# rossumur/espflix

Measured on AMD Instinct MI355X. Metric: MPEG-1 352x192 frames/s, higher is better.
Workload: dtype u8/int32; 1 GPU; 1024 streams/GPU x GOP(12) I+11P, 352x192 MPEG-1 ES resident in HBM, ids rank*1024.. per rank (BASELINE configs[2]; at 8 GPUs = configs[4], stream k on rank floor(k*8/8192)); streams_per_gpu=1024, streams_total=1024, es_bytes_per_gpu=46457181, parallelism=stream-partition x1, coefficients_per_gpu=44531885, ring_depth=2

## Files before the change

espflix_amd/csrc/efx_api.hip:

```cpp
#include <hip/hip_runtime.h>

#include <algorithm>
#include <memory>
#include <mutex>
#include <thread>

#include <cstdio>
#include <cstdlib>
#include <cstring>
#include <string>
#include <vector>

#include "efx.h"
#include "conform_sel.h"
#include "efx_internal.h"
#include "enc_core.h"
#include "import_px.h"
#include "crop_px.h"
#include "parse_tm.h"
#include "sbc_enc_core.h"
#include "trick_sel.h"

namespace efx {
struct DemuxChunk;
__global__ void k_demux_scan(const uint8_t*, const uint64_t*, const uint32_t*, const uint32_t*, DemuxChunk*);
__global__ void k_demux_offsets(const uint32_t*, const uint32_t*, DemuxChunk*, uint8_t*, const uint64_t*, uint32_t*, uint32_t*);
__global__ void k_demux(const uint8_t*, const uint64_t*, const uint32_t*, const uint32_t*, const DemuxChunk*, uint8_t*, PesEntry*);
__global__ void k_demux_fused(const uint8_t*, const uint64_t*, const uint32_t*, const uint32_t*, DemuxChunk*, uint8_t*, PesEntry*, uint32_t*, uint32_t*,
                              uint32_t*);
__global__ void k_demux_audio_scan(const uint8_t*, const uint64_t*, const uint32_t*, const uint32_t*, DemuxChunk*);
__global__ void k_demux_audio_offsets(const uint32_t*, const uint32_t*, DemuxChunk*, uint32_t*);
__global__ void k_demux_audio(const uint8_t*, const uint64_t*, const uint32_t*, const uint32_t*, const DemuxChunk*, uint8_t*, const uint64_t*);
__global__ void k_ts_sequences(const uint8_t*, const uint64_t*, const uint32_t*, const uint32_t*, PesEntry*, IdxInfo*);
__global__ void k_idx_bins(const PesEntry*, const uint32_t*, const IdxInfo*, uint32_t, uint32_t*, size_t);
__global__ void k_index(const uint8_t*, const uint64_t*, int, PicInfo*, SliceTmp*, uint32_t*, uint32_t*, uint32_t*,
                        const uint32_t*, const PesEntry*, const uint32_t*, const uint32_t*, int64_t*, int64_t*, int, int, int);
__global__ void k_advance(StreamState*, const uint32_t*, int64_t*, const int64_t*, int, int, int, int32_t*);
__global__ void k_slice_scan(const PicInfo*, const uint32_t*, int, int, const uint32_t*, uint32_t*, DecodeCounters*);
__global__ void k_slice_emit(const PicInfo*, const SliceTmp*, const uint32_t*, const uint64_t*, const uint32_t*, int, int,
                             const uint32_t*, SliceDesc*, uint32_t*);
__global__ void k_parse(const uint8_t*, const SliceDesc*, DecodeCounters*, const TmTables*, MbRec*, TmU4*, uint32_t*, uint32_t*,
                        int, int);
__global__ void k_recon(const MbRec*, const uint32_t*, const uint32_t*, const uint32_t*, uint8_t*, int, int, int, const int32_t*, int, int);
__global__ void k_recon_all(const MbRec*, const uint32_t*, const uint32_t*, const uint32_t*, uint8_t*, int, int, int, const int32_t*, int, int,
                            int, uint32_t*, uint32_t*, int);

__global__ void k_frame_hash(const uint8_t*, int, uint64_t*);
__global__ void k_fill(uint32_t*, uint32_t, size_t);
__global__ void k_composite(const uint8_t*, const VideoTables*, const VideoLineTemplates*, FieldArgs, uint16_t*);
__global__ void k_pdm(const int16_t*, int, int, int32_t*, uint16_t*);
template <int FMT, int CHROMA>
__global__ void k_export(const uint8_t*, int, ExportArgs);
__global__ void k_import_taps(ImportTap*, ImportArgs);
__global__ void k_import(const uint8_t*, uint8_t*, const ImportTap*, ImportArgs);
__global__ void k_crop_zero(CropArgs);
__global__ void k_crop_sums_i420(CropArgs);
__global__ void k_crop_sums_rgb24(CropArgs);
__global__ void k_crop_sums_rgbp(CropArgs);
__global__ void k_crop_rects(CropArgs);
template <int SOURCE>
__global__ void k_trick(TrickArgs);
__global__ void k_conform(ConformArgs);
__global__ void k_import_pcm(ImportPcmArgs);
__global__ void k_import_pcm_state(ImportPcmArgs);
__global__ void k_enc_begin(EncArgs);
__global__ void k_enc_act(EncArgs);
__global__ void k_enc_rows(EncArgs);
__global__ void k_enc_pack(EncArgs);
__global__ void k_sbc(const uint8_t*, size_t, int, int, SbcState*, const SbcTables*, int16_t*, size_t, uint32_t*, uint32_t*, int);
__global__ void k_sbc_frames(const uint8_t*, size_t, int, int, SbcFrameInfo*, uint32_t*, uint32_t*, SbcQueues*);
__global__ void k_sbc_plan(const SbcFrameInfo*, int, int, const SbcState*, SbcFramePlan*, uint32_t*, SbcQueues*, uint32_t*, int, int, uint32_t*,
                           uint32_t*, SbcExtraItem*, uint8_t*);
__global__ void k_sbc_par_stereo(const uint8_t*, size_t, int, int, const SbcState*, SbcState*, const SbcTables*, const SbcFrameInfo*, int16_t*,
                                 size_t, uint32_t*, int, SbcQueues*, const uint32_t*, int, const SbcExtraItem*, int);
__global__ void k_sbc_par_mono(const uint8_t*, size_t, int, int, const SbcState*, SbcState*, const SbcTables*, const SbcFrameInfo*, int16_t*,
                               size_t, uint32_t*, int, SbcQueues*, const uint32_t*, int, const SbcExtraItem*, int);
__global__ void k_sbc_gen(const uint8_t*, size_t, int, int, const SbcState*, SbcState*, const SbcTables*, const SbcFrameInfo*,
                          const SbcFramePlan*, int16_t*, size_t, int, SbcQueues*, const uint32_t*, int, const uint8_t*, int);
__global__ void k_sbc_finish(const uint8_t*, size_t, int, int, SbcState*, const SbcState*, const SbcTables*, int16_t*, size_t, uint32_t*,
                             uint32_t*, int, uint32_t*);
__global__ void k_sbc_enc(SbcEncArgs);
__global__ void k_sbc_enc_state(SbcEncArgs);
__global__ void k_mux(MuxArgs);
}

using namespace efx;

#ifndef EFX_SBC_WG_PER_CU
#define EFX_SBC_WG_PER_CU 4
#endif

#ifndef EFX_PARSE_STREAMS
#define EFX_PARSE_STREAMS 2
#endif
#ifndef EFX_SLOTS
#define EFX_SLOTS 3
#endif
constexpr int kParseStreams = EFX_PARSE_STREAMS;
constexpr int kMaxGroups = 16;
static_assert(kMaxGroups <= kExportMaxGroups, "k_export takes every reconstruction group of a call");
#ifndef EFX_RECON_MERGE
#define EFX_RECON_MERGE 1
#endif
constexpr int kReconMerge = EFX_RECON_MERGE;
#ifndef EFX_GROUP_STREAMS
#define EFX_GROUP_STREAMS 1024
#endif
constexpr int kGroupStreams = EFX_GROUP_STREAMS;
constexpr int kTimingRing = 64;
constexpr int kSlots = EFX_SLOTS;
constexpr int kUploads = 3;
constexpr size_t kReconSyncWords(size_t streams) { return (64 + streams) * 32; }

struct efx_ctx {
    efx_config cfg{};
    hipStream_t stream = nullptr;
    bool own_stream = false;
    bool pooled_streams = false;
    unsigned stream_serial = 0;
    std::string err;

    size_t es_cap = 0;
    bool decoded = false, results_valid = false;

    ParseTables* d_tables = nullptr;
    TmTables* d_tm_tables = nullptr;
    uint8_t* d_frames = nullptr;
    StreamState* d_state = nullptr;

    struct Upload {
        uint8_t* d_es = nullptr;
        uint64_t* d_stream_off = nullptr;
        uint32_t* d_stream_perm = nullptr;
        uint32_t* d_ts_len = nullptr;
        uint32_t* d_pkt_base = nullptr;
        uint32_t* d_es_len = nullptr;
        uint32_t* d_pes_count = nullptr;
        PesEntry* d_pes = nullptr;
        uint8_t* h_es = nullptr;
        uint8_t* h_meta = nullptr;
        std::vector<uint64_t> stream_off;
        std::vector<uint32_t> es_len;
        int n_streams = 0;
        int sort_groups = 1;
        size_t es_used = 0, ts_bytes = 0;
        bool ts_input = false, valid = false;
        hipEvent_t uploaded = nullptr;
        hipEvent_t last_read[kParseStreams] = {};
        hipEvent_t ev_demux[2] = {nullptr, nullptr};
        bool demux_timed = false;
    } up[kUploads];
    int cur_up = -1;
    struct Arena {
        uint8_t* base;
        size_t bytes;
        bool owned;
    };
    std::vector<Arena> arenas;
    hipStream_t copy_stream = nullptr;
    uint8_t* d_ts = nullptr;
    DemuxChunk* d_demux_chunks = nullptr;
    size_t pes_cap = 0;
    IdxInfo* d_idx_info = nullptr;
    uint64_t* d_ts_off = nullptr;
    uint32_t* d_idx_len = nullptr;
    uint32_t* d_idx_base = nullptr;
    PesEntry* d_idx_seq = nullptr;
    bool ts_ready = false;

    struct Slot {
        uint32_t* d_pic_count = nullptr;
        uint32_t* d_status = nullptr;
        DecodeCounters* d_counters = nullptr;
// ... 955 lines not shown
    bind_device(ctx);
    if (!ctx)
        return EFX_ERR_ARG;
    const size_t n = (size_t)ctx->cfg.max_streams;
    EFX_HIP(hipMemsetAsync(ctx->d_frames, 0, n * ctx->cfg.ring_depth * kFrameBytes, ctx->stream));
    std::vector<StreamState> init(n);
    for (auto& st : init) {
        st.fb_index = 1;
        st.pts_seen = 0;
        st.pts_carry = -1;
    }
    EFX_HIP(hipMemcpyAsync(ctx->d_state, init.data(), n * sizeof(StreamState), hipMemcpyHostToDevice, ctx->stream));
    EFX_HIP(hipStreamSynchronize(ctx->stream));
    ctx->recon_groups_unsynced = 0;
    return EFX_OK;
}

int efx_play_reset(efx_ctx* ctx)
{
    bind_device(ctx);
    if (!ctx)
        return EFX_ERR_ARG;
    int r = sync_all(ctx);
    if (r)
        return r;
    const size_t n = (size_t)ctx->cfg.max_streams;
    std::vector<StreamState> st(n);
    EFX_HIP(hipMemcpy(st.data(), ctx->d_state, n * sizeof(StreamState), hipMemcpyDeviceToHost));
    for (auto& x : st)
        x.pts_seen = 0;
    EFX_HIP(hipMemcpy(ctx->d_state, st.data(), n * sizeof(StreamState), hipMemcpyHostToDevice));
    return EFX_OK;
}

int efx_stream_state(efx_ctx* ctx, int stream, uint32_t* frame_index, int* pts_seen, int64_t* newest_pts)
{
    bind_device(ctx);
    if (!ctx || stream < 0 || stream >= ctx->cfg.max_streams)
        return EFX_ERR_ARG;
    int r = sync_all(ctx);
    if (r)
        return r;
    StreamState st;
    EFX_HIP(hipMemcpy(&st, ctx->d_state + stream, sizeof(st), hipMemcpyDeviceToHost));
    if (frame_index)
        *frame_index = st.fb_index;
    if (pts_seen)
        *pts_seen = (int)st.pts_seen;
    if (newest_pts)
        *newest_pts = st.pts_carry;
    return EFX_OK;
}

int efx_erase_frames(efx_ctx* ctx)
{
    bind_device(ctx);
    if (!ctx)
        return EFX_ERR_ARG;
    size_t bytes = (size_t)ctx->cfg.max_streams * ctx->cfg.ring_depth * kFrameBytes;
    EFX_HIP(hipMemsetAsync(ctx->d_frames, 0x30, bytes, ctx->stream));
    return EFX_OK;
}

int efx_decode_from(efx_ctx* ctx, int first_picture) { return efx_decode_range(ctx, first_picture, ctx ? ctx->cfg.max_pictures : 0); }

int efx_decode_range(efx_ctx* ctx, int first_picture, int n_pictures)
{
    bind_device(ctx);
    if (!ctx || first_picture < 0 || n_pictures < 1 || n_pictures > ctx->cfg.max_pictures)
        return EFX_ERR_ARG;
    if (ctx->cur_up < 0)
        return fail(ctx, EFX_ERR_STATE, "efx_decode: no streams uploaded");
    efx_ctx::Upload& u = ctx->up[ctx->cur_up];
    const int n_all = u.n_streams, P = ctx->cfg.max_pictures, D = ctx->cfg.ring_depth;
    const bool idle_at_call = ctx->recon_groups_unsynced == 0;
    const int G = ctx->opt_groups > 0 ? std::min(std::min(ctx->opt_groups, kMaxGroups), std::max(1, n_all / 8))
                                      : (idle_at_call ? group_count(n_all) : 1);
    {
        bool nested = true;
        for (int g = 1; g < G && nested; g++) {
            bool found = false;
            for (int k = 0; k <= u.sort_groups && !found; k++)
                found = group_first(n_all, u.sort_groups, k) == group_first(n_all, G, g);
            nested = found;
        }
        if (!nested) {
            int r = sync_all(ctx);
            if (r)
                return r;
            std::vector<uint32_t> perm((size_t)n_all);
            for (int i = 0; i < n_all; i++)
                perm[i] = (uint32_t)i;
            auto len_of = [&](uint32_t i) { return u.stream_off[i + 1] - u.stream_off[i]; };
            for (int g = 0; g < G; g++)
                std::stable_sort(perm.begin() + group_first(n_all, G, g), perm.begin() + group_first(n_all, G, g + 1),
                                 [&](uint32_t a, uint32_t b) { return len_of(a) > len_of(b); });
            EFX_HIP(hipMemcpy(u.d_stream_perm, perm.data(), perm.size() * sizeof(uint32_t), hipMemcpyHostToDevice));
            u.sort_groups = G;
        }
    }
    hipStream_t sr = ctx->stream;
    int timing_slot = -1;
    if (ctx->timing && !ctx->timing_ring.empty()) {
        timing_slot = (int)(ctx->timed_calls++ % kTimingRing);
        ctx->timing_groups[timing_slot] = (uint8_t)G;
        ctx->timing_leaders[timing_slot] = 0;
        ctx->timing_launches[timing_slot] = (uint16_t)(((G + kReconMerge - 1) / kReconMerge) * (ctx->opt_recon_mode == 0 ? n_pictures : 1));
    }
    ctx->last_upload = ctx->cur_up;
    ctx->last_n_streams = u.n_streams;
    ctx->last_ts_input = u.ts_input;
    const int R = (G + kReconMerge - 1) / kReconMerge;
    ctx->n_groups = R;
    for (int r = 0; r < R; r++) {
        const int h0 = r * kReconMerge, h1 = std::min(G, h0 + kReconMerge);
        const int rs0 = group_first(n_all, G, h0), rn = group_first(n_all, G, h1) - rs0;
        const int slot = (int)(ctx->subcalls++ % kSlots);
        ctx->groups[r] = {slot, rs0, rn, h0, h1 - h0};
        efx_ctx::Slot& sl = ctx->slot[slot];
        sl.upload = ctx->cur_up;
        const bool wrap = ++sl.epoch > 255;
        if (wrap)
            sl.epoch = 1;
        efx_ctx::TimingEvents* te0 = nullptr;
        for (int g = h0; g < h1; g++) {
            const int s0 = group_first(n_all, G, g), n = group_first(n_all, G, g + 1) - s0;
            const int pi = (int)(ctx->parse_calls++ % kParseStreams);
            hipStream_t sp = ctx->parse_streams[pi];
            DecodeCounters* counters = sl.d_counters + g;
            uint32_t* slice_base = sl.d_slice_base + (size_t)s0 * P + g;
            SliceDesc* descs = sl.d_descs + (size_t)s0 * P * kMaxSlicesPerPicture;

            EFX_HIP(hipStreamWaitEvent(sp, u.uploaded, 0));
            EFX_HIP(hipStreamWaitEvent(sp, sl.recon_done, 0));
            if (wrap && g == h0) {
                EFX_HIP(hipMemsetAsync(sl.d_mbrecs, 0, (size_t)ctx->cfg.max_streams * P * kMbCount * sizeof(MbRec), sp));
                EFX_HIP(hipEventRecord(sl.wrap_cleared, sp));
            } else if (wrap)
                EFX_HIP(hipStreamWaitEvent(sp, sl.wrap_cleared, 0));
            efx_ctx::TimingEvents* te = timing_slot >= 0 ? &ctx->timing_ring[(size_t)timing_slot * kMaxGroups + g] : nullptr;
            if (te && !te->ev[0])
                for (auto& ev : te->ev)
                    EFX_HIP(hipEventCreate(&ev));
            if (g == h0)
                te0 = te;
            if (te)
                EFX_HIP(hipEventRecord(te->ev[0], sp));
            hipLaunchKernelGGL(k_index, dim3(n), dim3(64 * kIndexWaves), 0, sp, u.d_es, u.d_stream_off, P, sl.d_pics, sl.d_slices_tmp,
                               sl.d_pic_count, sl.d_status, sl.d_qtab, ctx->d_tables->scan, u.d_pes, u.d_pkt_base, u.d_pes_count,
                               u.ts_input ? sl.d_pts : nullptr, u.ts_input ? sl.d_pts + (size_t)ctx->cfg.max_streams * P : nullptr,
                               first_picture, s0, n_pictures);
            hipLaunchKernelGGL(k_slice_scan, dim3(1), dim3(1024), 0, sp, sl.d_pics, sl.d_pic_count, n, P, u.d_stream_perm + s0,
                               slice_base, counters);
            hipLaunchKernelGGL(k_slice_emit, dim3((n * P * kMaxSlicesPerPicture + 255) / 256), dim3(256), 0, sp, sl.d_pics,
                               sl.d_slices_tmp, sl.d_pic_count, u.d_stream_off, slice_base, n, P, u.d_stream_perm + s0, descs, sl.d_status);
            if (te)
                EFX_HIP(hipEventRecord(te->ev[1], sp));
            const int max_slices = n * P * kMaxSlicesPerPicture;
            const int parse_waves = (max_slices + kParseLanes - 1) / kParseLanes;
            int parse_wgs = (parse_waves + kParseWaves - 1) / kParseWaves;
            const bool recon_busy = ctx->opt_parse_cap == 1 || (ctx->opt_parse_cap == 0 && ctx->recon_groups_unsynced > 0);
            if (ctx->parse_wg_cap > 0 && recon_busy)
                parse_wgs = std::min(parse_wgs, ctx->parse_wg_cap);
            hipLaunchKernelGGL(k_parse, dim3(parse_wgs), dim3(64 * kParseWaves), 0, sp, u.d_es,
                               descs, counters, ctx->d_tm_tables, sl.d_mbrecs, sl.d_raw, sl.d_coefs, sl.d_status, P, sl.epoch);
            if (te)
                EFX_HIP(hipEventRecord(te->ev[2], sp));
            EFX_HIP(hipEventRecord(sl.parse_done[g - h0], sp));
            EFX_HIP(hipEventRecord(u.last_read[pi], sp));
        }

        for (int g = h0; g < h1; g++)
            EFX_HIP(hipStreamWaitEvent(sr, sl.parse_done[g - h0], 0));
        if (te0) {
            EFX_HIP(hipEventRecord(te0->ev[4], sr));
            ctx->timing_leaders[timing_slot] |= (uint16_t)(1u << h0);
        }
        hipLaunchKernelGGL(k_advance, dim3((rn + 255) / 256), dim3(256), 0, sr, ctx->d_state, sl.d_pic_count,
                           u.ts_input ? sl.d_pts : nullptr, u.ts_input ? sl.d_pts + (size_t)ctx->cfg.max_streams * P : nullptr, rs0, rn,
                           P, sl.d_call_pos);
        constexpr int kGroupsPerPicture = (kMbCount * 6 + 63) / 64;
#ifdef EFX_RECON_ITEMS2
        constexpr int kReconGridY = (kGroupsPerPicture + 1) / 2;
#else
        constexpr int kReconGridY = kGroupsPerPicture;
#endif
        if (ctx->opt_recon_mode == 0) {
            for (int p = 0; p < n_pictures; p++)
                hipLaunchKernelGGL(k_recon, dim3(rn, kReconGridY), dim3(64), 0, sr, sl.d_mbrecs, sl.d_coefs,
                                   ctx->d_tables->scan, sl.d_qtab, ctx->d_frames, P, D, p, sl.d_call_pos, sl.epoch, rs0);
        } else if (rn > 0) {
            EFX_HIP(hipMemsetAsync(sl.d_recon_sync, 0, kReconSyncWords((size_t)rn) * sizeof(uint32_t), sr));
            const long long items = (long long)rn * kGroupsPerPicture * n_pictures;
            const int per_cu = ctx->opt_recon_waves > 0 ? ctx->opt_recon_waves : 18;
            const long long waves = ctx->opt_recon_items > 0 ? (items + ctx->opt_recon_items - 1) / ctx->opt_recon_items
                                                             : std::min<long long>(items, (long long)ctx->n_cus * per_cu);
            hipLaunchKernelGGL(k_recon_all, dim3((unsigned)waves), dim3(64), 0, sr, sl.d_mbrecs,
                               sl.d_coefs, ctx->d_tables->scan, sl.d_qtab, ctx->d_frames, P, D, n_pictures, sl.d_call_pos, sl.epoch, rs0, rn,
                               sl.d_recon_sync, sl.d_status, ctx->opt_recon_items);
        }
        if (te0)
            EFX_HIP(hipEventRecord(te0->ev[3], sr));
        EFX_HIP(hipEventRecord(sl.recon_done, sr));
        ctx->last_recon_done = sl.recon_done;
        ctx->recon_groups_unsynced++;
    }
    EFX_HIP(hipGetLastError());
    ctx->decoded = true;
    ctx->results_valid = false;
    return EFX_OK;
}

int efx_decode(efx_ctx* ctx) { return efx_decode_from(ctx, 0); }

int efx_sync(efx_ctx* ctx)
{
    bind_device(ctx);
    if (!ctx)
        return EFX_ERR_ARG;
    return sync_all(ctx);
}

static int fetch_results(efx_ctx* ctx)
{
    if (!ctx->decoded)
        return fail(ctx, EFX_ERR_STATE, "no decode has run");
    if (ctx->results_valid)
        return EFX_OK;
    int r = sync_all(ctx);
    if (r)
        return r;
    const bool ts_input = ctx->last_ts_input;
    ctx->n_streams = ctx->last_n_streams;
    const size_t P = (size_t)ctx->cfg.max_pictures;
    ctx->h_pic_count.resize(ctx->n_streams);
    ctx->h_status.resize(ctx->n_streams);
    ctx->h_call_pos.resize(2 * (size_t)ctx->n_streams);
    if (ts_input)
        ctx->h_pts.resize((size_t)ctx->n_streams * P);
    else
        ctx->h_pts.clear();
    ctx->h_counters = DecodeCounters{};
    for (int g = 0; g < ctx->n_groups; g++) {
        const efx_ctx::Group& gr = ctx->groups[g];
        const efx_ctx::Slot& sl = ctx->slot[gr.slot];
        const size_t f = (size_t)gr.first, c = (size_t)gr.count;
        if (!c)
            continue;
        EFX_HIP(hipMemcpy(ctx->h_pic_count.data() + f, sl.d_pic_count + f, c * sizeof(uint32_t), hipMemcpyDeviceToHost));
        EFX_HIP(hipMemcpy(ctx->h_status.data() + f, sl.d_status + f, c * sizeof(uint32_t), hipMemcpyDeviceToHost));
        EFX_HIP(hipMemcpy(ctx->h_call_pos.data() + 2 * f, sl.d_call_pos + 2 * f, 2 * c * sizeof(int32_t), hipMemcpyDeviceToHost));
        if (ts_input)
            EFX_HIP(hipMemcpy(ctx->h_pts.data() + f * P, sl.d_pts + f * P, c * P * sizeof(int64_t), hipMemcpyDeviceToHost));
        for (int h = gr.half0; h < gr.half0 + gr.halves; h++) {
            DecodeCounters dc;
            EFX_HIP(hipMemcpy(&dc, sl.d_counters + h, sizeof(dc), hipMemcpyDeviceToHost));
            ctx->h_counters.total_slices += dc.total_slices;
            ctx->h_counters.coefficients += dc.coefficients;
            ctx->h_counters.macroblocks += dc.macroblocks;
        }
    }
    ctx->results_valid = true;
    return EFX_OK;
}

int efx_picture_count(efx_ctx* ctx, int stream, int* n_pictures)
{
    bind_device(ctx);
    if (!ctx || !n_pictures || stream < 0)
        return EFX_ERR_ARG;
    int r = fetch_results(ctx);
    if (r)
        return r;
    if (stream >= ctx->n_streams)
        return EFX_ERR_ARG;
    *n_pictures = (int)ctx->h_pic_count[stream];
    return EFX_OK;
}

int efx_stream_status(efx_ctx* ctx, int stream, uint32_t* bits)
{
    bind_device(ctx);
    if (!ctx || !bits || stream < 0)
        return EFX_ERR_ARG;
    int r = fetch_results(ctx);
    if (r)
        return r;
    if (stream >= ctx->n_streams)
        return EFX_ERR_ARG;
    *bits = ctx->h_status[stream];
    return EFX_OK;
}

int efx_picture_pts(efx_ctx* ctx, int stream, int picture, int64_t* pts)
{
    bind_device(ctx);
    if (!ctx || !pts || stream < 0 || picture < 0)
        return EFX_ERR_ARG;
    int r = fetch_results(ctx);
    if (r)
        return r;
    if (stream >= ctx->n_streams)
        return EFX_ERR_ARG;
    if (ctx->h_pts.empty()) {
        *pts = picture;
        return EFX_OK;
    }
// ... 1356 lines not shown
```

espflix_amd/csrc/k_index.hip:

```cpp
#include <hip/hip_runtime.h>

#include "efx_internal.h"
#include "efx.h"

namespace efx {

namespace {

__device__ inline uint32_t wave_excl_scan(uint32_t v, uint32_t* total)
{
    uint32_t x = v;
    int lane = threadIdx.x & 63;
#pragma unroll
    for (int d = 1; d < 64; d <<= 1) {
        uint32_t y = __shfl_up(x, d, 64);
        if (lane >= d)
            x += y;
    }
    *total = __shfl(x, 63, 64);
    return x - v;
}

__device__ inline uint32_t load_bits(const uint8_t* p, uint32_t bitpos, int n)
{
    const uint8_t* q = p + (bitpos >> 3);
    uint32_t w = ((uint32_t)q[0] << 24) | ((uint32_t)q[1] << 16) | ((uint32_t)q[2] << 8) | q[3];
    return (w << (bitpos & 7)) >> (32 - n);
}

__device__ inline bool hunt_arrives(const uint8_t* base, uint32_t bit, uint32_t next_off)
{
    const uint32_t target = next_off * 8;
    for (int step = 0; step < 4096; step++) {
        uint32_t f = bit;
        {
            uint32_t by = f >> 3;
            uint32_t v = (uint32_t)base[by] & (0xFFu >> (f & 7));
            while (!v && by + 1 < next_off) {
                by++;
                v = base[by];
            }
            if (!v)
                return false;
            f = by * 8 + (uint32_t)(__clz((int)v) - 24);
        }
        const uint32_t at = f - bit >= 24 ? f - 23 : bit;
        if (at + 32 == target)
            return true;
        if (at + 32 > target)
            return false;
        const uint32_t m = load_bits(base, at + 24, 8);
        if (m < 0x0E || m == 0xB3 || m == 0xB7 || m == 0xB8)
            return false;
        bit = at + 32;
    }
    return false;
}

}

__global__ __launch_bounds__(64 * kIndexWaves) void k_index(
    const uint8_t* __restrict__ es, const uint64_t* __restrict__ stream_off, int max_pictures, PicInfo* __restrict__ pics,
    SliceTmp* __restrict__ slices_tmp, uint32_t* __restrict__ pic_count, uint32_t* __restrict__ status, uint32_t* __restrict__ qtab,
    const uint32_t* __restrict__ scan_tab, const PesEntry* __restrict__ pes, const uint32_t* __restrict__ pkt_base,
    const uint32_t* __restrict__ pes_count, int64_t* __restrict__ pts_out, int64_t* __restrict__ pts_newest, int first_picture,
    int stream0, int pic_limit)
{
    __shared__ uint32_t u_off[kMaxUnitsPerStream];
    __shared__ uint32_t u_info[kMaxUnitsPerStream];
    __shared__ uint32_t sh_misc[5];
    __shared__ uint32_t w_tot[kIndexWaves][4];
    constexpr int kKbPerWave = 16, kKbPerRound = kKbPerWave * kIndexWaves;
    static_assert(kKbPerRound == 64, "one wave scans the kilobyte counts of a round: one per lane");
    __shared__ uint32_t kb_count[kKbPerRound];
    __shared__ uint32_t round_total;

    const int s = stream0 + blockIdx.x;
    const int tid = threadIdx.x, lane = tid & 63, wave = tid >> 6;
    const uint8_t* base = es + stream_off[s];
    const uint32_t len = (uint32_t)(stream_off[s + 1] - stream_off[s]);

    uint32_t n_units = 0;
    constexpr int kUnroll = 4;
    for (uint32_t round = 0; round < len; round += kKbPerRound * 1024) {
        uint32_t mask[kKbPerWave];
        uint32_t before2[kKbPerWave / 2];
        const uint32_t wave_base = round + wave * kKbPerWave * 1024;
#pragma unroll
        for (int k = 0; k < kKbPerWave / kUnroll; k++) {
            if (wave_base + k * kUnroll * 1024 >= len) {
#pragma unroll
                for (int u = 0; u < kUnroll; u++)
                    mask[k * kUnroll + u] = 0;
#pragma unroll
                for (int h = 0; h < kUnroll / 2; h++)
                    before2[(k * kUnroll) / 2 + h] = 0;
                if (lane < kUnroll)
                    kb_count[wave * kKbPerWave + k * kUnroll + lane] = 0;
                continue;
            }
            uint32_t wv[kUnroll][5];
#pragma unroll
            for (int u = 0; u < kUnroll; u++) {
                const uint32_t pos = wave_base + (k * kUnroll + u) * 1024 + lane * 16;
                const uint8_t* p = base + (pos < len ? pos : 0);
                uint4 d = *reinterpret_cast<const uint4*>(p);
                wv[u][0] = d.x;
                wv[u][1] = d.y;
                wv[u][2] = d.z;
                wv[u][3] = d.w;
                wv[u][4] = *reinterpret_cast<const uint32_t*>(p + 16);
            }
#pragma unroll
            for (int u = 0; u < kUnroll; u++) {
                const uint32_t pos = wave_base + (k * kUnroll + u) * 1024 + lane * 16;
                uint32_t* w = wv[u];
                if (pos + 16 >= len)
                    w[4] = 0;
                uint32_t m = 0;
#pragma unroll
                for (int i = 0; i < 16; i++) {
                    uint32_t lo = w[i >> 2], hi = w[(i >> 2) + 1];
                    uint32_t v = (i & 3) ? __builtin_amdgcn_alignbyte(hi, lo, i & 3) : lo;
                    if ((v & 0xFFFFFF) == 0x010000)
                        m |= 1u << i;
                }
                mask[k * kUnroll + u] = pos < len ? m : 0u;
            }
#pragma unroll
            for (int h = 0; h < kUnroll / 2; h++) {
                const int kb = k * kUnroll + 2 * h;
                uint32_t t2;
                before2[kb / 2] = wave_excl_scan(__popc(mask[kb]) | (__popc(mask[kb + 1]) << 16), &t2);
                if (lane == 0) {
                    kb_count[wave * kKbPerWave + kb] = t2 & 0xFFFF;
                    kb_count[wave * kKbPerWave + kb + 1] = t2 >> 16;
                }
            }
        }
        __syncthreads();
        if (wave == 0) {
            uint32_t tot;
            const uint32_t ex = wave_excl_scan(kb_count[lane], &tot);
            kb_count[lane] = ex;
            if (lane == 0)
                round_total = tot;
        }
        __syncthreads();
#pragma unroll
        for (int kb = 0; kb < kKbPerWave; kb++) {
            uint32_t m = mask[kb];
            uint32_t idx = n_units + kb_count[wave * kKbPerWave + kb] + ((before2[kb / 2] >> (16 * (kb & 1))) & 0xFFFF);
            const uint32_t pos = wave_base + kb * 1024 + lane * 16;
            while (m) {
                const int i = __ffs(m) - 1;
                m &= m - 1;
// ... 145 lines not shown
                if (seg < (uint32_t)kMaxSlicesPerPicture) {
                    const uint32_t next = (i + 1 < n_units) ? u_off[i + 1] - 4 : len;
                    SliceTmp t;
                    t.off = u_off[i];
                    t.len_code = ((next - u_off[i]) << 8) | code;
                    myslices[open * kMaxSlicesPerPicture + seg] = t;
                } else
                    my_st |= EFX_STREAM_TRUNCATED;
            }
        }
        if (my_st)
            atomicOr(&sh_misc[4], my_st);
    }
    __syncthreads();
    if (tid == 0)
        status[s] = st | sh_misc[4];
    __syncthreads();

    uint32_t npics = sh_misc[0];

    if (pts_out) {
        const PesEntry* mp = pes + pkt_base[s];
        uint32_t np = pes_count[s];
        if (np & kDemuxFailedFlag) {
            np = 0;
            if (tid == 0)
                atomicOr(&status[s], EFX_STREAM_INTERNAL);
        }
        if (tid == 0)
            pts_newest[s] = np ? mp[np - 1].pts : kNoPts;
        for (uint32_t p = tid; p < npics; p += 64 * kIndexWaves) {
            const uint32_t limit = mypics[p].start_off + 1;
            uint32_t a = 0, b = np;
            while (a < b) {
                uint32_t m = (a + b) >> 1;
                if (mp[m].es_off <= limit)
                    a = m + 1;
                else
                    b = m;
            }
            pts_out[(size_t)s * max_pictures + p] = a ? mp[a - 1].pts : -1;
        }
    }

    for (uint32_t p = wave; p < npics; p += kIndexWaves) {
        PicInfo pi = mypics[p];
        if (!pi.custom_q)
            continue;
        uint32_t flags = pi.reserved;
        const uint8_t* sp = base + pi.seq_off;
        uint32_t intra_bit = 63, non_intra_bit = (flags & 1) ? 64 + 512 : 64;
        uint32_t t = scan_tab[lane];
        uint32_t zz = t & 0xFF;
        uint32_t qi = (flags & 1) ? load_bits(sp, intra_bit + 8 * zz, 8) : ((t >> 16) & 0xFF);
        uint32_t qn = (flags & 2) ? load_bits(sp, non_intra_bit + 8 * zz, 8) : 16;
        qtab[((size_t)s * max_pictures + p) * 64 + lane] = (t & 0xFFFF) | (qi << 16) | (qn << 24);
    }
}

__global__ void k_advance(StreamState* __restrict__ state, const uint32_t* __restrict__ pic_count, int64_t* __restrict__ pts,
                          const int64_t* __restrict__ pts_newest, int stream0, int n_streams, int max_pictures,
                          int32_t* __restrict__ call_pos)
{
    const int t = blockIdx.x * blockDim.x + threadIdx.x;
    if (t >= n_streams)
        return;
    const int s = stream0 + t;
    StreamState st = state[s];
    const int n = (int)pic_count[s];
    int f = st.pts_seen ? -1 : n;
    if (pts) {
        int64_t* my = pts + (size_t)s * max_pictures;
        for (int i = 0; i < n; i++) {
            if (my[i] == -1 && st.pts_carry != -1)
                my[i] = st.pts_carry;
            if (f == n && my[i] != -1)
                f = i;
        }
        if (pts_newest[s] != kNoPts)
            st.pts_carry = pts_newest[s];
    } else if (!st.pts_seen)
        f = 0;
    call_pos[2 * s] = (int32_t)st.fb_index;
    call_pos[2 * s + 1] = f;
    if (n > 0) {
        st.fb_index += f < 0 ? (uint32_t)n : (uint32_t)(n - 1 > f ? n - 1 - f : 0);
        if (f < n)
            st.pts_seen = 1;
    }
    state[s] = st;
}

__global__ __launch_bounds__(1024) void k_slice_scan(const PicInfo* __restrict__ pics,
                                                     const uint32_t* __restrict__ pic_count, int n_streams,
                                                     int max_pictures, const uint32_t* __restrict__ stream_perm,
                                                     uint32_t* __restrict__ slice_base,
                                                     DecodeCounters* __restrict__ counters)
{
    __shared__ uint32_t wave_tot[16];
    __shared__ uint32_t carry;
    constexpr int kRun = 4;
    const int tid = threadIdx.x, lane = tid & 63, wv = tid >> 6;
    const int n = n_streams * max_pictures;
    if (tid == 0)
        carry = 0;
    __syncthreads();
    for (int base = 0; base < n; base += 1024 * kRun) {
        uint32_t v[kRun];
#pragma unroll
        for (int r = 0; r < kRun; r++) {
            const int i = base + tid * kRun + r;
            v[r] = 0;
            if (i < n) {
                int p = i / n_streams, s = (int)stream_perm[i - p * n_streams];
                if ((uint32_t)p < pic_count[s])
                    v[r] = pics[(size_t)s * max_pictures + p].n_slices;
            }
        }
        uint32_t mine = 0;
#pragma unroll
        for (int r = 0; r < kRun; r++)
            mine += v[r];
        uint32_t tot;
        uint32_t ex = wave_excl_scan(mine, &tot);
        if (lane == 63)
            wave_tot[wv] = tot;
        __syncthreads();
        uint32_t off = carry;
        for (int k = 0; k < wv; k++)
            off += wave_tot[k];
        uint32_t at = off + ex;
#pragma unroll
        for (int r = 0; r < kRun; r++) {
            const int i = base + tid * kRun + r;
            if (i < n)
                slice_base[i] = at;
            at += v[r];
        }
        __syncthreads();
        if (tid == 1023)
            carry = at;
        __syncthreads();
    }
    if (tid == 0) {
        counters->total_slices = carry;
        counters->streams = (uint32_t)n_streams;
        counters->coefficients = 0;
        counters->macroblocks = 0;
        counters->next_wave = 0;
        slice_base[n] = carry;
    }
}

__global__ __launch_bounds__(256) void k_slice_emit(const PicInfo* __restrict__ pics,
                                                    const SliceTmp* __restrict__ slices_tmp,
                                                    const uint32_t* __restrict__ pic_count,
                                                    const uint64_t* __restrict__ stream_off,
                                                    const uint32_t* __restrict__ slice_base, int n_streams,
                                                    int max_pictures, const uint32_t* __restrict__ stream_perm,
                                                    SliceDesc* __restrict__ descs, uint32_t* __restrict__ status)
{
    int t = blockIdx.x * blockDim.x + threadIdx.x;
    int k = t % kMaxSlicesPerPicture, i = t / kMaxSlicesPerPicture;
    if (i >= n_streams * max_pictures)
        return;
    int p = i / n_streams, s = (int)stream_perm[i - p * n_streams];
    if ((uint32_t)p >= pic_count[s])
        return;
    PicInfo pi = pics[(size_t)s * max_pictures + p];
    if (k >= pi.n_slices)
        return;
    SliceTmp st = slices_tmp[(size_t)s * max_pictures * kMaxSlicesPerPicture + pi.first_slice + k];
    SliceDesc d;
    d.es_off = (uint32_t)stream_off[s] + st.off;
    d.es_len = st.len_code >> 8;
    d.stream = (uint32_t)s;
    d.pic_code_flags = (uint32_t)p | ((st.len_code & 0xFF) << 8) | ((uint32_t)pi.type << 16) | ((uint32_t)pi.full_pel << 18) |
                       ((uint32_t)pi.r_size << 19) | ((uint32_t)pi.custom_q << 22);
    uint32_t limit = kMbCount;
    bool out_of_order = false;
    {
        const uint32_t code = st.len_code & 0xFF;
        const SliceTmp* all = slices_tmp + (size_t)s * max_pictures * kMaxSlicesPerPicture + pi.first_slice;
        for (int j = 0; j < (int)pi.n_slices; j++) {
            const uint32_t other = all[j].len_code & 0xFF;
            if (other > code && (other - 1) * kMbW < limit)
                limit = (other - 1) * kMbW;
            if (other == code && j > k)
                limit = 0;
            out_of_order |= j < k && other >= code;
        }
    }
    if (out_of_order)
        atomicOr(&status[s], EFX_STREAM_SLICE_ORDER);
    d.mb_limit = limit;
    d.reserved = 0;
    descs[slice_base[i] + k] = d;
}

}
```

Measured before the change: 9.037 million frames/s.

## Sort slice descriptors by length within 64-stream runs for parse load balance

Restructures k_slice_emit so each block handles one picture index across 64 streams. It computes keys from slice byte length in shared memory and writes descriptors in descending-length order within that run, using a rank by linear count. The intent is that k_parse waves pick up similarly sized slices together, which reduces divergence and tail imbalance. The cost is a per-thread O(n) rank over up to 1024 keys in the emit kernel, and descriptors are no longer in stream order within a run.

```diff
diff --git a/espflix_amd/csrc/efx_api.hip b/espflix_amd/csrc/efx_api.hip
--- a/espflix_amd/csrc/efx_api.hip
+++ b/espflix_amd/csrc/efx_api.hip
@@ -19,6 +19,7 @@
 #include "crop_px.h"
 #include "parse_tm.h"
 #include "sbc_enc_core.h"
+#include "slice_order.h"
 #include "trick_sel.h"
 
 namespace efx {
@@ -1280,7 +1281,7 @@
                                first_picture, s0, n_pictures);
             hipLaunchKernelGGL(k_slice_scan, dim3(1), dim3(1024), 0, sp, sl.d_pics, sl.d_pic_count, n, P, u.d_stream_perm + s0,
                                slice_base, counters);
-            hipLaunchKernelGGL(k_slice_emit, dim3((n * P * kMaxSlicesPerPicture + 255) / 256), dim3(256), 0, sp, sl.d_pics,
+            hipLaunchKernelGGL(k_slice_emit, dim3((n + kSliceRunPairs - 1) / kSliceRunPairs, P), dim3(sord::kRunSlots), 0, sp, sl.d_pics,
                                sl.d_slices_tmp, sl.d_pic_count, u.d_stream_off, slice_base, n, P, u.d_stream_perm + s0, descs, sl.d_status);
             if (te)
                 EFX_HIP(hipEventRecord(te->ev[1], sp));
diff --git a/espflix_amd/csrc/k_index.hip b/espflix_amd/csrc/k_index.hip
--- a/espflix_amd/csrc/k_index.hip
+++ b/espflix_amd/csrc/k_index.hip
@@ -2,6 +2,7 @@
 
 #include "efx_internal.h"
 #include "efx.h"
+#include "slice_order.h"
 
 namespace efx {
 
@@ -453,50 +454,71 @@
     }
 }
 
-__global__ __launch_bounds__(256) void k_slice_emit(const PicInfo* __restrict__ pics,
-                                                    const SliceTmp* __restrict__ slices_tmp,
-                                                    const uint32_t* __restrict__ pic_count,
-                                                    const uint64_t* __restrict__ stream_off,
-                                                    const uint32_t* __restrict__ slice_base, int n_streams,
-                                                    int max_pictures, const uint32_t* __restrict__ stream_perm,
-                                                    SliceDesc* __restrict__ descs, uint32_t* __restrict__ status)
-{
-    int t = blockIdx.x * blockDim.x + threadIdx.x;
-    int k = t % kMaxSlicesPerPicture, i = t / kMaxSlicesPerPicture;
-    if (i >= n_streams * max_pictures)
+__global__ __launch_bounds__(sord::kRunSlots) void k_slice_emit(const PicInfo* __restrict__ pics,
+                                                                const SliceTmp* __restrict__ slices_tmp,
+                                                                const uint32_t* __restrict__ pic_count,
+                                                                const uint64_t* __restrict__ stream_off,
+                                                                const uint32_t* __restrict__ slice_base, int n_streams,
+                                                                int max_pictures, const uint32_t* __restrict__ stream_perm,
+                                                                SliceDesc* __restrict__ descs, uint32_t* __restrict__ status)
+{
+    static_assert(sord::kSlotsPerPair == kMaxSlicesPerPicture, "slice_order.h numbers a run's slots by pair and slice");
+    __shared__ uint64_t keys[sord::kRunSlots];
+    __shared__ uint32_t most_slices;
+    const int t = threadIdx.x, k = t % kMaxSlicesPerPicture, j = t / kMaxSlicesPerPicture;
+    const int p = blockIdx.y, pos0 = blockIdx.x * kSliceRunPairs, pos = pos0 + j;
+    if (t == 0)
+        most_slices = 0;
+    __syncthreads();
+    bool has_slice = false;
+    int s = 0;
+    PicInfo pi = {};
+    if (pos < n_streams) {
+        s = (int)stream_perm[pos];
+        if ((uint32_t)p < pic_count[s]) {
+            pi = pics[(size_t)s * max_pictures + p];
+            has_slice = k < pi.n_slices;
+            if (k == 0 && pi.n_slices)
+                atomicMax(&most_slices, (uint32_t)pi.n_slices);
+        }
+    }
+    SliceDesc d = {};
+    if (has_slice) {
+        SliceTmp st = slices_tmp[(size_t)s * max_pictures * kMaxSlicesPerPicture + pi.first_slice + k];
+        d.es_off = (uint32_t)stream_off[s] + st.off;
+        d.es_len = st.len_code >> 8;
+        d.stream = (uint32_t)s;
+        d.pic_code_flags = (uint32_t)p | ((st.len_code & 0xFF) << 8) | ((uint32_t)pi.type << 16) | ((uint32_t)pi.full_pel << 18) |
+                           ((uint32_t)pi.r_size << 19) | ((uint32_t)pi.custom_q << 22);
+        uint32_t limit = kMbCount;
+        bool out_of_order = false;
+        {
+            const uint32_t code = st.len_code & 0xFF;
+            const SliceTmp* all = slices_tmp + (size_t)s * max_pictures * kMaxSlicesPerPicture + pi.first_slice;
+            for (int o = 0; o < (int)pi.n_slices; o++) {
+                const uint32_t other = all[o].len_code & 0xFF;
+                if (other > code && (other - 1) * kMbW < limit)
+                    limit = (other - 1) * kMbW;
+                if (other == code && o > k)
+                    limit = 0;
+                out_of_order |= o < k && other >= code;
+            }
+        }
+        if (out_of_order)
+            atomicOr(&status[s], EFX_STREAM_SLICE_ORDER);
+        d.mb_limit = limit;
+        d.reserved = 0;
+    }
+    const uint64_t mine = sord::key(has_slice, d.es_len, (uint32_t)t);
+    keys[k * kSliceRunPairs + j] = mine;
+    __syncthreads();
+    if (!has_slice)
         return;
-    int p = i / n_streams, s = (int)stream_perm[i - p * n_streams];
-    if ((uint32_t)p >= pic_count[s])
-        return;
-    PicInfo pi = pics[(size_t)s * max_pictures + p];
-    if (k >= pi.n_slices)
-        return;
-    SliceTmp st = slices_tmp[(size_t)s * max_pictures * kMaxSlicesPerPicture + pi.first_slice + k];
-    SliceDesc d;
-    d.es_off = (uint32_t)stream_off[s] + st.off;
-    d.es_len = st.len_code >> 8;
-    d.stream = (uint32_t)s;
-    d.pic_code_flags = (uint32_t)p | ((st.len_code & 0xFF) << 8) | ((uint32_t)pi.type << 16) | ((uint32_t)pi.full_pel << 18) |
-                       ((uint32_t)pi.r_size << 19) | ((uint32_t)pi.custom_q << 22);
-    uint32_t limit = kMbCount;
-    bool out_of_order = false;
-    {
-        const uint32_t code = st.len_code & 0xFF;
-        const SliceTmp* all = slices_tmp + (size_t)s * max_pictures * kMaxSlicesPerPicture + pi.first_slice;
-        for (int j = 0; j < (int)pi.n_slices; j++) {
-            const uint32_t other = all[j].len_code & 0xFF;
-            if (other > code && (other - 1) * kMbW < limit)
-                limit = (other - 1) * kMbW;
-            if (other == code && j > k)
-                limit = 0;
-            out_of_order |= j < k && other >= code;
-        }
-    }
-    if (out_of_order)
-        atomicOr(&status[s], EFX_STREAM_SLICE_ORDER);
-    d.mb_limit = limit;
-    d.reserved = 0;
-    descs[slice_base[i] + k] = d;
-}
-
-}
+    const int pair0 = p * n_streams + pos0, pair1 = p * n_streams + min(pos0 + kSliceRunPairs, n_streams);
+    const uint32_t base = slice_base[pair0], count = slice_base[pair1] - base;
+    const uint32_t r = sord::rank(keys, most_slices * kSliceRunPairs, mine);
+    if (r < count)
+        descs[base + r] = d;
+}
+
+}
diff --git a/espflix_amd/csrc/slice_order.h b/espflix_amd/csrc/slice_order.h
--- /dev/null
+++ b/espflix_amd/csrc/slice_order.h
@@ -0,0 +1,37 @@
+#pragma once
+#include <stdint.h>
+
+#if defined(__HIPCC__)
+#define EFX_SORD_HD __host__ __device__
+#else
+#define EFX_SORD_HD
+#endif
+
+namespace efx {
+
+constexpr int kSliceRunPairs = 64;
+
+namespace sord {
+
+constexpr int kSlotsPerPair = 16;
+constexpr int kRunSlots = kSliceRunPairs * kSlotsPerPair;
+constexpr uint32_t kMaxLen = (1u << 24) - 1;
+
+EFX_SORD_HD inline uint64_t key(bool has_slice, uint32_t es_len, uint32_t t)
+{
+    return has_slice ? ((uint64_t)es_len << 11) | (uint64_t)(kRunSlots - t) : 0u;
+}
+
+EFX_SORD_HD inline uint32_t rank(const uint64_t* keys, uint32_t n, uint64_t mine)
+{
+    uint32_t r = 0;
+#if defined(__HIP_DEVICE_COMPILE__)
+#pragma unroll 8
+#endif
+    for (uint32_t j = 0; j < n; j++)
+        r += keys[j] > mine ? 1u : 0u;
+    return r;
+}
+
+}
+}
```

New measurement: 9.259 million frames/s, median of 6. 1.02x the previous value.
